# hyeeiin/ECG-Multimodal-Model

Hardware: AMD Instinct MI355X
Metric: samples/sec fwd+bwd, batch-256 multimodal (img+sig+clin), 1->8 MI355X (higher is better)
Workload: dtype bf16; 1 GPU; full multimodal (image 3x224x224 + 5000-pt signal + 16-dim clinical), fwd+bwd+Adam, encoders unfrozen; image_hw=224x224, per_gpu_batch=256, global_batch=256, parallelism=dp1

## Files before the change

### ecg-multimodal-model_amd/csrc/api.hip

```cpp
#include <stdarg.h>

#include "ops.h"

static thread_local char g_err[512] = "";

void ecg_set_error(const char* fmt, ...) {
  va_list ap;
  va_start(ap, fmt);
  vsnprintf(g_err, sizeof(g_err), fmt, ap);
  va_end(ap);
}

static inline ConvGeom geom_of(const ecgmm_conv_desc* c) {
  return make_geom(c->N, c->H, c->W, c->Cin, c->Cout, c->R, c->S, c->stride, c->pad_h, c->pad_w);
}
#define S_(x) ((hipStream_t)(x))

extern "C" {

int ecgmm_version(void) { return ECGMM_VERSION; }
const char* ecgmm_last_error(void) { return g_err; }

const char* ecgmm_switch_name(int i) { return i >= 0 && i < sw::COUNT ? sw::ALL[i]->env : nullptr; }
int ecgmm_switch_get(const char* env_name, int64_t* value) {
  Switch* s = sw::find(env_name);
  if (!s) ECG_FAIL(ECGMM_ERR_SHAPE, "switch_get: unknown switch %s", env_name ? env_name : "(null)");
  if (!value) ECG_FAIL(ECGMM_ERR_SHAPE, "switch_get: null value pointer");
  *value = s->get();
  return 0;
}
int ecgmm_switch_set(const char* env_name, int64_t value) {
  Switch* s = sw::find(env_name);
  if (!s) ECG_FAIL(ECGMM_ERR_SHAPE, "switch_set: unknown switch %s", env_name ? env_name : "(null)");
  if (s == &sw::SIDE_WGRAD)
    ECG_FAIL(ECGMM_ERR_SHAPE, "switch_set: ECGMM_SIDE_WGRAD is each plan's own state after start-up, call ecgmm_side_wgrad()");
  if (!s->runtime) ECG_FAIL(ECGMM_ERR_SHAPE, "switch_set: %s is read once at start-up", s->env);
  s->set((long)value);
  return 0;
}
int ecgmm_conv_halo_enable(int on) { sw::CONV_HALO.set(on); return 0; }
int ecgmm_conv_halo_cus(int cus) { sw::HALO_CUS.set(cus); return 0; }
int ecgmm_conv_halo_w4(int on) { sw::HALO_W4.set(on); return 0; }
int ecgmm_conv_halo_stagger(int on) { sw::HALO_STAGGER.set(on); return 0; }
int ecgmm_conv_halo_stream(int on) { sw::HALO_STREAM.set(on); return 0; }
int ecgmm_conv_halo_pingpong(int on) { sw::HALO_PP.set(on); return 0; }
int ecgmm_conv_wgrad_pingpong(int on) { sw::WGRAD_PP.set(on); return 0; }
int ecgmm_conv_wgrad_ring_enable(int on) { sw::WGRAD_RING.set(on); return 0; }
int ecgmm_bn_fold(int on) { sw::BN_FOLD.set(on); return 0; }
int ecgmm_bn_fold_slice(int on) { sw::BN_FOLD_SLICE.set(on); return 0; }
int ecgmm_bn_fuse_min_pixels(int64_t m) { sw::BN_FUSE_MIN_M.set((long)m); return 0; }
int ecgmm_stem_recompute(int on) { sw::STEM_RECOMPUTE.set(on); return 0; }
int ecgmm_infer_down_side(int on) { sw::INFER_DOWN_SIDE.set(on); return 0; }

int ecgmm_nchw_to_nhwc(int dtype, const float* src, void* dst, int N, int C, int64_t HW, void* stream) {
  return ecg_nchw_to_nhwc(dtype, src, dst, N, C, (long)HW, S_(stream));
}
int ecgmm_nhwc_to_nchw(int dtype, const void* src, float* dst, int N, int C, int64_t HW, void* stream) {
  return ecg_nhwc_to_nchw(dtype, src, dst, N, C, (long)HW, S_(stream));
}
int ecgmm_cast(int dtype, const float* src, void* dst, int64_t n, void* stream) {
  return ecg_cast(dtype, src, dst, (long)n, S_(stream));
}
int ecgmm_uncast(int dtype, const void* src, float* dst, int64_t n, void* stream) {
  return ecg_uncast(dtype, src, dst, (long)n, S_(stream));
}
int ecgmm_pack_conv_weight(int dtype, const float* w, void* fwd, void* dgrad, int Cout, int Cin, int RS,
                           void* stream) {
  return ecg_pack_weight(dtype, w, fwd, dgrad, Cout, Cin, RS, S_(stream));
}

int ecgmm_conv_stats_rows(int64_t out_pixels) { return ecg_conv_stats_rows((long)out_pixels); }
int ecgmm_conv_fwd(int dtype, const ecgmm_conv_desc* c, const void* x, const void* w_fwd, const float* bias, void* y,
                   float* stats, int act, void* stream) {
  return ecg_conv_igemm(dtype, 0, geom_of(c), x, w_fwd, y, bias, nullptr, stats, act, S_(stream));
}
int ecgmm_conv_bwd_data(int dtype, const ecgmm_conv_desc* c, const void* dy, const void* w_dgrad, const void* addend,
                        void* dx, void* stream) {
  return ecg_conv_igemm(dtype, 1, geom_of(c), dy, w_dgrad, dx, nullptr, addend, nullptr, 0, S_(stream));
}
size_t ecgmm_conv_bwd_weight_workspace(int dtype, const ecgmm_conv_desc* c) {
  return ecg_conv_wgrad_workspace(dtype, geom_of(c));
}
int ecgmm_conv_bwd_weight(int dtype, const ecgmm_conv_desc* c, const void* x, const void* dy, float* dw, int accumulate,
                          void* ws, size_t ws_bytes, void* stream) {
  return ecg_conv_wgrad(dtype, geom_of(c), x, dy, dw, accumulate, ws, ws_bytes, S_(stream));
}

size_t ecgmm_stem_packed_elems(int Cin, int R) { return ecg_stem_packed_elems(Cin, R); }
int ecgmm_stem_stats_rows(int N, int Cin, int H, int W, int R) { return ecg_stem_stats_rows(N, Cin, H, W, R); }
int ecgmm_stem_pack(int dtype, const float* w, void* packed, int Cin, int R, void* stream) {
  return ecg_stem_pack(dtype, w, packed, Cin, R, S_(stream));
}
int ecgmm_stem_fwd(int dtype, const float* x, const void* packed, const float* bias, void* y, float* stats, int N,
// ... 319 lines not shown
```

### ecg-multimodal-model_amd/csrc/conv_igemm.hip

```cpp
#include "ops.h"

namespace {

template <typename T> struct Mma;
template <> struct Mma<bf16_t> {
  static __device__ __forceinline__ void run(f32x4& acc, const u32x4& a, const u32x4& b) {
    acc = __builtin_amdgcn_mfma_f32_16x16x32_bf16(__builtin_bit_cast(bf16x8_t, a), __builtin_bit_cast(bf16x8_t, b),
                                                  acc, 0, 0, 0);
  }
};
template <> struct Mma<float> {
  static __device__ __forceinline__ void run(f32x4& acc, const u32x4& a, const u32x4& b) {
#pragma unroll
    for (int j = 0; j < 4; ++j)
      acc = __builtin_amdgcn_mfma_f32_16x16x4f32(__uint_as_float(a[j]), __uint_as_float(b[j]), acc, 0, 0, 0);
  }
};

__device__ __forceinline__ void dma16(__amdgpu_buffer_rsrc_t rs, unsigned char* lds_wave_base, unsigned voffset) {
#if defined(__HIP_DEVICE_COMPILE__)
  __builtin_amdgcn_raw_ptr_buffer_load_lds(rs, (__attribute__((address_space(3))) void*)lds_wave_base, 16, voffset, 0, 0,
                                           0);
#endif
}
// ... 514 lines not shown
static inline double conv_flops(const ConvGeom& g) {
  return 2.0 * (double)g.N * g.OH * g.OW * g.Cout * g.R * g.S * g.Cin;
}

int ecg_conv_igemm(int dtype, int mode, const ConvGeom& g, const void* src, const void* wpk, void* dst,
                   const float* bias, const void* addend, float* stats, int act, hipStream_t stream, ConvEpi* epi) {
  IgemmParams p;
  memset(&p, 0, sizeof(p));
  p.src = src; p.wpk = wpk; p.dst = dst; p.bias = bias; p.addend = addend; p.stats = stats; p.act = act;
  p.Nimg = g.N; p.R = g.R; p.S = g.S; p.stride = g.stride; p.pad_h = g.pad_h; p.pad_w = g.pad_w;
  if (mode == 0) {
    p.Hs = g.H; p.Ws = g.W; p.Cs = g.Cin; p.Hd = g.OH; p.Wd = g.OW; p.Cd = g.Cout;
  } else {
    p.Hs = g.OH; p.Ws = g.OW; p.Cs = g.Cout; p.Hd = g.H; p.Wd = g.W; p.Cd = g.Cin;
  }
  long M = (long)g.N * p.Hd * p.Wd;
  if (M <= 0 || M > 0x7fffffffL) ECG_FAIL(ECGMM_ERR_SHAPE, "conv: pixel count %ld out of range", M);
  {
    auto magic = [](unsigned d, unsigned& m, unsigned& sh) {
      if (d < 1) d = 1;
      int l = 0;
      while ((1u << l) < d) ++l;
      m = (unsigned)(((1ull << (31 + l)) + d - 1) / d);
      sh = 31 + l;
    };
    const bool par = mode == 1 && g.stride == 2;
    for (int c = 0; c < 4; ++c) {
      const int ph_ = par ? c >> 1 : 0, pw_ = par ? c & 1 : 0;
      const int Hc_ = par ? (p.Hd - ph_ + 1) >> 1 : p.Hd, Wc_ = par ? (p.Wd - pw_ + 1) >> 1 : p.Wd;
      magic((unsigned)(Hc_ * Wc_), p.mul_hw[c], p.sh_hw[c]);
      magic((unsigned)Wc_, p.mul_w[c], p.sh_w[c]);
    }
  }
  p.M = (int)M;
  const int vec = dtype == ECGMM_BF16 ? 8 : 4;
  if (p.Cs % vec != 0) ECG_FAIL(ECGMM_ERR_SHAPE, "conv: reduction channels %d not a multiple of %d", p.Cs, vec);
  if (dtype != ECGMM_BF16 && dtype != ECGMM_F32) ECG_FAIL(ECGMM_ERR_DTYPE, "conv: bad dtype %d", dtype);
  {
    const double esz = (double)dtype_size(dtype);
    double bytes = esz * ((double)g.N * p.Hs * p.Ws * p.Cs + (double)M * p.Cd * (addend ? 2.0 : 1.0) +
                          (double)g.R * g.S * g.Cin * g.Cout);
    if (epi && epi->red_y) bytes += esz * (double)M * p.Cd * (epi->red_mask ? 2.0 : 1.0);
    if (epi && epi->src2 && mode == 1 && g.stride == 2) bytes += esz * ((double)g.N * p.Hs * p.Ws * p.Cs + (double)g.Cin * g.Cout);
    ecg_prof_begin(dtype == ECGMM_F32 ? (mode == 0 ? ECG_PROF_IGEMM_F32_FWD : ECG_PROF_IGEMM_F32_DGRAD)
                                      : (mode == 0 ? ECG_PROF_IGEMM_FWD : ECG_PROF_IGEMM_DGRAD),
                   conv_flops(g), bytes, stream);
  }
  if (epi) epi->src2_done = 0;
  if (epi && epi->src2 && mode == 1 && g.stride == 2 && g.pad_h <= 1 && g.pad_w <= 1 && !addend) {
    p.src2 = epi->src2; p.wpk2 = epi->wpk2;
    epi->src2_done = 1;
  }
  int rc;
  if (ecg_conv_halo_ok(dtype, mode, g)) {
    rc = ecg_conv_halo(mode, g, src, wpk, dst, bias, addend, stats, act, epi, stream);
  } else {
    if (epi) {
      epi->stats_rows = ecg_conv_stats_rows(M);
      epi->red_done = 0;
      epi->red_rows_n = 0;
    }
    rc = dtype == ECGMM_BF16 ? launch_T<bf16_t>(p, mode, stream) : launch_T<float>(p, mode, stream);
  }
  ecg_prof_end(stream);
  return rc;
}
```

### ecg-multimodal-model_amd/csrc/ops.h

```cpp
#pragma once
#include "common.h"
#include "switches.h"

int ecg_conv_stats_rows(long M);
struct ConvEpi {
  const void* red_y;
  const void* red_mask;
  const float* red_coef;
  float* red_rows;
  int wg_rows;
  const void* src2;
  const void* wpk2;
  int src2_done;
  int stats_rows;
  int red_done;
  int red_rows_n;
};
int ecg_conv_igemm(int dtype, int mode, const ConvGeom& g, const void* src, const void* wpk, void* dst,
                   const float* bias, const void* addend, float* stats, int act, hipStream_t stream,
                   ConvEpi* epi = nullptr);
bool ecg_conv_halo_ok(int dtype, int mode, const ConvGeom& g);
int ecg_conv_halo_rows(int mode, const ConvGeom& g);
int ecg_conv_halo(int mode, const ConvGeom& g, const void* src, const void* wpk, void* dst, const float* bias,
                  const void* addend, float* stats, int act, ConvEpi* epi, hipStream_t stream);
size_t ecg_conv_wgrad_workspace(int dtype, const ConvGeom& g);
void ecg_conv_wgrad_narrow(bool narrow, int slots = 256);
int ecg_conv_wgrad(int dtype, const ConvGeom& g, const void* x, const void* dy, float* grad_oihw, int accumulate,
                   void* workspace, size_t workspace_bytes, hipStream_t stream);
size_t ecg_stem_packed_elems(int Cin, int R);
int ecg_stem_stats_rows(int N, int Cin, int H, int W, int R);
int ecg_stem_pack(int dtype, const float* w, void* out, int Cin, int R, hipStream_t stream);
int ecg_stem_fwd(int dtype, const float* x, const void* wpk, const float* bias, void* y, float* stats, int N, int Cin,
                 int H, int W, int R, hipStream_t stream);
size_t ecg_stem_wgrad_workspace(int N, int Cin, int H, int W, int R);
int ecg_stem_wgrad(int dtype, const float* x, const void* dy, float* grad, int accumulate, void* workspace,
                   size_t workspace_bytes, int N, int Cin, int H, int W, int R, hipStream_t stream);
int ecg_stem_stats_only_rows(int N, int Cin, int H, int W, int R);
int ecg_stem_wg_stats_rows(int N, int Cin, int H, int W, int R);
int ecg_stem_fwd_wgrows(int dtype, const float* x, const void* wpk, const float* bias, void* y, float* stats, int N, int Cin,
                        int H, int W, int R, hipStream_t stream);
int ecg_stem_stats_only(int dtype, const float* x, const void* wpk, const float* bias, float* stats, int N, int Cin, int H,
                        int W, int R, hipStream_t stream);
int ecg_stem_wgrad_reduce(const float* slab, float* grad, int rows, int NG, int accumulate, hipStream_t stream);
int ecg_stem_dgrad(int dtype, const void* dy, const float* w, float* dx, int N, int Cin, int H, int W, int R,
                   hipStream_t stream);
bool ecg_stem_fused_ok(int dtype, int Cin, int R);
int ecg_stem_pool_fwd(const float* x, const void* wpk, const float* coef, void* pooled, unsigned char* idx, int N, int Cin,
                      int H, int W, hipStream_t stream);
size_t ecg_stem_pool_bwd_workspace(int N, int Cin, int H, int W);
int ecg_stem_pool_bwd(const float* x, const void* wpk, const float* coef, const float* gamma, const void* dp, const void* pooled,
                      const unsigned char* idx, float* dgamma, float* dbeta, float* dw, void* ws, size_t ws_bytes, int N,
                      int Cin, int H, int W, hipStream_t stream);
int ecg_pool_bn_bwd_reduce(int dtype, const void* dp, const void* pooled, const float* coef, const float* gamma, float* dgamma,
                           float* dbeta, int N, int H, int W, int C, float* scratch, const float** bcoef_out,
                           hipStream_t stream);
int ecg_bn_rows(int dtype, long M, int C);
int ecg_bn_finalize(const float* partial, int rows, int C, double count, const float* gamma, const float* beta,
                    float* rm, float* rv, long long* nbt, float momentum, float eps, float* coef, hipStream_t stream);
int ecg_bn_eval_coef(int C, const float* gamma, const float* beta, const float* rm, const float* rv, float eps,
                     float* coef, hipStream_t stream);
int ecg_col_stats(int dtype, const void* x, long M, int C, float* partial, int* rows_out, hipStream_t stream);
struct EcgBnFold {
  const float* partial; int rows; double count;
  const float* gamma; const float* beta;
  float* rm; float* rv; long long* nbt;
  float momentum, eps;
};
bool ecg_bn_fold_ok(int C, int rows);
int ecg_bn_act_fold(int dtype, const void* y, float* coef, const EcgBnFold& f, const void* res, const float* rcoef,
                    const float* gate, int rows_per_sample, int relu, void* out, long M, int C, hipStream_t stream,
                    unsigned char* relu_bits = nullptr);
int ecg_bn_act(int dtype, const void* y, const float* coef, const void* res, const float* rcoef, const float* gate,
               int rows_per_sample, int relu, void* out, long M, int C, hipStream_t stream, unsigned char* relu_bits = nullptr);
size_t ecg_bn_bwd_scratch(int dtype, long M, int C);
int ecg_bn_bwd(int dtype, const void* dout, const void* maskref, const float* gate, const float* addc,
               int rows_per_sample, const void* y, const float* coef, const float* gamma, float* dgamma, float* dbeta,
               void* dy, void* dz_out, float* dbias, long M, int C, float* scratch, hipStream_t stream,
// ... 170 lines not shown
```

### ecg-multimodal-model_amd/hip/lib.py

```python
import ctypes as C
import os

F32, BF16 = 0, 1
ACT_NONE, ACT_RELU, ACT_SIGMOID = 0, 1, 2
RESNET18_NPARAMS, RESNET18_NBUFFERS = 62, 60
RESNET1D_NPARAMS, RESNET1D_NBUFFERS = 52, 27

_PKG_DIR = os.path.dirname(os.path.dirname(os.path.abspath(__file__)))
LIB_PATH = os.environ.get("ECGMM_LIB") or os.path.join(_PKG_DIR, "libecgmm_hip.so")

vp, i32, i64, u64, f32, f64, sz = C.c_void_p, C.c_int, C.c_int64, C.c_uint64, C.c_float, C.c_double, C.c_size_t


class ConvDesc(C.Structure):
    _fields_ = [(n, i32) for n in ("N", "H", "W", "Cin", "Cout", "R", "S", "stride", "pad_h", "pad_w")]


class ResNet18Desc(C.Structure):
    _fields_ = [("N", i32), ("H", i32), ("W", i32), ("out_dim", i32), ("dtype", i32), ("training", i32),
                ("bn_momentum", f32), ("bn_eps", f32)]


class ResNet1DDesc(C.Structure):
    _fields_ = [("N", i32), ("cin", i32), ("L", i32), ("num_classes", i32), ("dtype", i32), ("training", i32),
                ("bn_momentum", f32), ("bn_eps", f32), ("dropout_p", f32), ("seed", u64), ("offset", u64)]


class HeadDesc(C.Structure):
    _fields_ = [("B", i32), ("dim", i32 * 3), ("hidden", i32), ("num_classes", i32), ("training", i32),
                ("ln_eps", f32), ("dropout_p", f32), ("seed", u64), ("offset", u64)]


class LSTMDesc(C.Structure):
    _fields_ = [(n, i32) for n in ("B", "T", "In", "H", "layers", "bidirectional", "batch_first", "save_for_backward")]


class CRNNFrontDesc(C.Structure):
    _fields_ = [("B", i32), ("F", i32), ("T", i32), ("dtype", i32), ("training", i32), ("bn_momentum", f32), ("bn_eps", f32)]


P = C.POINTER
SIGNATURES = {
    "ecgmm_version": (i32, []),
    "ecgmm_last_error": (C.c_char_p, []),
    "ecgmm_switch_name": (C.c_char_p, [i32]),
    "ecgmm_switch_get": (i32, [C.c_char_p, P(i64)]),
    "ecgmm_switch_set": (i32, [C.c_char_p, i64]),
    "ecgmm_resnet18_fwd_workspace": (sz, [P(ResNet18Desc)]),
    "ecgmm_resnet18_bwd_workspace": (sz, [P(ResNet18Desc)]),
    "ecgmm_resnet18_forward": (i32, [P(ResNet18Desc), vp, P(vp), P(vp), vp, vp, sz, vp]),
    "ecgmm_resnet18_backward": (i32, [P(ResNet18Desc), vp, vp, P(vp), P(vp), vp, vp, sz, i32, i32, vp]),
    "ecgmm_resnet18_backward_dx": (i32, [P(ResNet18Desc), vp, vp, P(vp), P(vp), vp, vp, sz, i32, i32, vp, vp]),
    "ecgmm_resnet18_gradcam": (i32, [P(ResNet18Desc), vp, P(vp), vp, vp, sz, vp, vp]),
    "ecgmm_head_fwd_workspace": (sz, [P(HeadDesc)]),
    "ecgmm_head_bwd_workspace": (sz, [P(HeadDesc)]),
    "ecgmm_head_forward": (i32, [P(HeadDesc), P(vp), P(vp), P(vp), vp, vp, vp, sz, vp]),
    "ecgmm_head_backward": (i32, [P(HeadDesc), P(vp), P(vp), P(vp), P(vp), vp, P(vp), vp, vp, sz, vp]),
    "ecgmm_conv_halo_enable": (i32, [i32]),
    "ecgmm_conv_halo_cus": (i32, [i32]),
    "ecgmm_conv_halo_w4": (i32, [i32]),
    "ecgmm_conv_halo_stagger": (i32, [i32]),
    "ecgmm_conv_halo_stream": (i32, [i32]),
    "ecgmm_conv_halo_pingpong": (i32, [i32]),
    "ecgmm_conv_wgrad_pingpong": (i32, [i32]),
    "ecgmm_conv_wgrad_ring_enable": (i32, [i32]),
    "ecgmm_side_wgrad": (i32, [i32]),
    "ecgmm_side_defer_join": (i32, [i32]),
    "ecgmm_resnet1d_side_wgrad": (i32, [i32]),
    "ecgmm_side_wait": (i32, [vp]),
    "ecgmm_side_stream": (vp, []),
    "ecgmm_side_fork": (i32, [vp]),
    "ecgmm_resnet1d_fwd_workspace": (sz, [P(ResNet1DDesc)]),
    "ecgmm_resnet1d_bwd_workspace": (sz, [P(ResNet1DDesc)]),
    "ecgmm_resnet1d_forward": (i32, [P(ResNet1DDesc), vp, P(vp), P(vp), vp, vp, sz, vp]),
    "ecgmm_resnet1d_backward": (i32, [P(ResNet1DDesc), vp, vp, P(vp), P(vp), vp, vp, sz, i32, i32, vp]),
    "ecgmm_resnet1d_backward_dx": (i32, [P(ResNet1DDesc), vp, vp, P(vp), P(vp), vp, vp, sz, i32, i32, vp, vp]),
    "ecgmm_resnet1d_gradcam": (i32, [P(ResNet1DDesc), vp, P(vp), vp, vp, sz, vp, vp]),
    "ecgmm_nchw_to_nhwc": (i32, [i32, vp, vp, i32, i32, i64, vp]),
    "ecgmm_nhwc_to_nchw": (i32, [i32, vp, vp, i32, i32, i64, vp]),
    "ecgmm_cast": (i32, [i32, vp, vp, i64, vp]),
    "ecgmm_uncast": (i32, [i32, vp, vp, i64, vp]),
    "ecgmm_pack_conv_weight": (i32, [i32, vp, vp, vp, i32, i32, i32, vp]),
    "ecgmm_conv_stats_rows": (i32, [i64]),
    "ecgmm_conv_fwd": (i32, [i32, P(ConvDesc), vp, vp, vp, vp, vp, i32, vp]),
    "ecgmm_conv_fwd_wgrows": (i32, [i32, P(ConvDesc), vp, vp, vp, vp, vp, vp, i32, vp]),
    "ecgmm_conv_bwd_data": (i32, [i32, P(ConvDesc), vp, vp, vp, vp, vp]),
    "ecgmm_conv_bwd_weight_workspace": (sz, [i32, P(ConvDesc)]),
    "ecgmm_conv_bwd_weight": (i32, [i32, P(ConvDesc), vp, vp, vp, i32, vp, sz, vp]),
    "ecgmm_stem_packed_elems": (sz, [i32, i32]),
    "ecgmm_stem_stats_rows": (i32, [i32, i32, i32, i32, i32]),
    "ecgmm_stem_pack": (i32, [i32, vp, vp, i32, i32, vp]),
    "ecgmm_stem_fwd": (i32, [i32, vp, vp, vp, vp, vp, i32, i32, i32, i32, i32, vp]),
    "ecgmm_stem_wg_stats_rows": (i32, [i32, i32, i32, i32, i32]),
    "ecgmm_stem_fwd_wgrows": (i32, [i32, vp, vp, vp, vp, vp, i32, i32, i32, i32, i32, vp]),
    "ecgmm_stem_stats_only_rows": (i32, [i32, i32, i32, i32, i32]),
    "ecgmm_stem_stats_only": (i32, [i32, vp, vp, vp, vp, i32, i32, i32, i32, i32, vp]),
    "ecgmm_stem_pool_fwd": (i32, [vp, vp, vp, vp, vp, i32, i32, i32, i32, vp]),
    "ecgmm_stem_pool_bwd_workspace": (sz, [i32, i32, i32, i32]),
    "ecgmm_stem_pool_bwd": (i32, [vp, vp, vp, vp, vp, vp, vp, vp, vp, vp, vp, sz, i32, i32, i32, i32, vp]),
    "ecgmm_stem_bwd_weight_workspace": (sz, [i32, i32, i32, i32, i32]),
    "ecgmm_stem_bwd_weight": (i32, [i32, vp, vp, vp, i32, vp, sz, i32, i32, i32, i32, i32, vp]),
    "ecgmm_stem_bwd_data": (i32, [i32, vp, vp, vp, i32, i32, i32, i32, i32, vp]),
    "ecgmm_col_stats_rows": (i32, [i32, i64, i32]),
    "ecgmm_col_stats": (i32, [i32, vp, i64, i32, vp, vp]),
    "ecgmm_bn_finalize": (i32, [vp, i32, i32, f64, vp, vp, vp, vp, vp, f32, f32, vp, vp]),
    "ecgmm_bn_eval_coef": (i32, [i32, vp, vp, vp, vp, f32, vp, vp]),
    "ecgmm_bn_act": (i32, [i32, vp, vp, vp, vp, vp, i32, i32, vp, i64, i32, vp]),
    "ecgmm_bn_act_from_rows": (i32, [i32, vp, vp, i32, f64, vp, vp, vp, vp, vp, f32, f32, vp, vp, vp, vp, i32, i32, vp, i64, i32, vp]),
    "ecgmm_bn_bwd_scratch": (sz, [i32, i64, i32]),
    "ecgmm_bn_bwd": (i32, [i32, vp, vp, vp, vp, i32, vp, vp, vp, vp, vp, vp, vp, vp, i64, i32, vp, vp]),
    "ecgmm_bn_eval_bwd": (i32, [i32, vp, vp, vp, vp, i32, vp, vp, vp, vp, vp, vp, vp, i64, i32, vp, vp]),
# ... 37 lines not shown
    "ecgmm_signal_preprocess": (i32, [vp, vp, i32, i32, vp, vp, i32, P(f64), P(f64), P(f64), i32, vp, sz, vp]),
    "ecgmm_signal_filter_zscore": (i32, [vp, vp, i32, i32, P(f64), P(f64), P(f64), i32, i32, f64, vp]),
    "ecgmm_signal_gather_augment": (i32, [vp, i64, i32, vp, i32, vp, vp, i32, f32, f32, f32, f32, i32, i32, u64, u64, vp]),
    "ecgmm_glu_fwd": (i32, [vp, vp, i64, i32, vp]),
    "ecgmm_glu_bwd": (i32, [vp, vp, vp, i64, i32, vp]),
    "ecgmm_sparsemax_fwd": (i32, [vp, vp, i64, i32, vp]),
    "ecgmm_sparsemax_bwd": (i32, [vp, vp, vp, i64, i32, vp]),
    "ecgmm_ew": (i32, [i32, vp, vp, vp, i64, f32, vp]),
    "ecgmm_split_cols": (i32, [vp, vp, vp, i64, i32, i32, i32, vp]),
    "ecgmm_split_cols_bwd": (i32, [vp, vp, vp, vp, i64, i32, i32, i32, vp]),
    "ecgmm_bn_small_fwd": (i32, [vp, vp, vp, vp, vp, vp, vp, vp, i32, i32, i32, f32, f32, vp]),
    "ecgmm_bn_small_bwd": (i32, [vp, vp, vp, vp, vp, vp, vp, i32, i32, i32, vp]),
    "ecgmm_bn_small_eval_bwd": (i32, [vp, vp, vp, vp, vp, vp, vp, i32, i32, i32, vp]),
    "ecgmm_entropy_fwd": (i32, [vp, vp, i64, i32, f32, vp]),
    "ecgmm_entropy_bwd": (i32, [vp, vp, vp, i64, i32, f32, vp]),
    "ecgmm_image_resize_tables_bytes": (sz, [i32, i32, i32, i32]),
    "ecgmm_image_resize_tables": (i32, [i32, i32, i32, i32, vp, sz]),
    "ecgmm_image_transform": (i32, [vp, vp, i32, i32, i32, i32, i32, vp, sz, P(f32), P(f32), vp]),
    "ecgmm_resnet18_infer_prepared_bytes": (sz, [P(ResNet18Desc)]),
    "ecgmm_resnet18_infer_prepare": (i32, [P(ResNet18Desc), P(vp), P(vp), vp, sz, vp]),
    "ecgmm_resnet18_infer_workspace": (sz, [P(ResNet18Desc)]),
    "ecgmm_resnet18_infer": (i32, [P(ResNet18Desc), vp, vp, sz, vp, vp, sz, vp]),
    "ecgmm_resnet1d_infer_prepared_bytes": (sz, [P(ResNet1DDesc)]),
    "ecgmm_resnet1d_infer_prepare": (i32, [P(ResNet1DDesc), P(vp), P(vp), vp, sz, vp]),
    "ecgmm_resnet1d_infer_workspace": (sz, [P(ResNet1DDesc)]),
    "ecgmm_resnet1d_infer": (i32, [P(ResNet1DDesc), vp, vp, sz, vp, vp, sz, vp]),
    "ecgmm_infer_down_side": (i32, [i32]),
    "ecgmm_conv_fwd_fused": (i32, [i32, P(ConvDesc), vp, vp, vp, vp, vp, i32, vp]),
    "ecgmm_fold_conv_bn": (i32, [i32, i32, vp, vp, vp, vp, vp, vp, f32, vp, vp, vp, i32, i32, i32, vp]),
    "ecgmm_relu_maxpool": (i32, [i32, vp, vp, i32, i32, i32, i32, vp]),
    "ecgmm_gate_res_relu": (i32, [i32, vp, vp, vp, vp, i64, i32, i32, vp]),
    "ecgmm_prof_enable": (i32, [i32]),
    "ecgmm_prof_pause": (i32, [i32]),
    "ecgmm_prof_collect": (i32, [i32, P(f64), P(f64), P(f64), P(i64)]),
    "ecgmm_lstm_fwd_workspace": (sz, [P(LSTMDesc)]),
    "ecgmm_lstm_bwd_workspace": (sz, [P(LSTMDesc)]),
    "ecgmm_lstm_forward": (i32, [P(LSTMDesc), vp, P(vp), vp, vp, vp, vp, vp, vp, sz, vp]),
    "ecgmm_lstm_backward": (i32, [P(LSTMDesc), vp, P(vp), vp, vp, vp, vp, vp, vp, vp, P(vp), vp, vp, vp, sz, vp]),
    "ecgmm_conv5_in1_stats_rows": (i32, [i32, i32, i32]),
    "ecgmm_conv5_in1_fwd": (i32, [i32, vp, vp, vp, vp, vp, i32, i32, i32, vp]),
    "ecgmm_conv5_in1_bwd_weight_workspace": (sz, [i32, i32, i32]),
    "ecgmm_conv5_in1_bwd_weight": (i32, [i32, vp, vp, vp, vp, i32, vp, sz, i32, i32, i32, vp]),
    "ecgmm_conv5_bwd_weight_workspace": (sz, [i32, P(ConvDesc)]),
    "ecgmm_conv5_bwd_weight": (i32, [i32, P(ConvDesc), vp, vp, vp, i32, vp, sz, vp]),
    "ecgmm_bnrelu_maxpool2": (i32, [i32, vp, vp, vp, vp, i32, i32, i32, i32, i32, vp]),
    "ecgmm_pool2_bn_bwd_workspace": (sz, [i32, i32, i32, i32]),
    "ecgmm_pool2_bn_bwd": (i32, [i32, vp, vp, vp, vp, i32, vp, vp, vp, vp, i32, i32, i32, i32, i32, vp, sz, vp]),
    "ecgmm_crnn_front_fwd_workspace": (sz, [P(CRNNFrontDesc)]),
    "ecgmm_crnn_front_bwd_workspace": (sz, [P(CRNNFrontDesc)]),
    "ecgmm_crnn_front_forward": (i32, [P(CRNNFrontDesc), vp, P(vp), P(vp), vp, vp, sz, vp]),
    "ecgmm_crnn_front_backward": (i32, [P(CRNNFrontDesc), vp, vp, P(vp), P(vp), vp, vp, sz, vp]),
}

LATER_SYMBOLS = ("ecgmm_resnet18_backward_dx", "ecgmm_resnet18_gradcam", "ecgmm_resnet1d_backward_dx",
                 "ecgmm_resnet1d_gradcam", "ecgmm_stem_bwd_data", "ecgmm_bn_eval_bwd", "ecgmm_bn_small_eval_bwd",
                 "ecgmm_resnet18_infer_prepared_bytes", "ecgmm_resnet18_infer_prepare", "ecgmm_resnet18_infer_workspace",
                 "ecgmm_resnet18_infer", "ecgmm_resnet1d_infer_prepared_bytes", "ecgmm_resnet1d_infer_prepare",
                 "ecgmm_resnet1d_infer_workspace", "ecgmm_resnet1d_infer", "ecgmm_infer_down_side", "ecgmm_conv_fwd_fused",
                 "ecgmm_fold_conv_bn", "ecgmm_relu_maxpool", "ecgmm_gate_res_relu",
                 "ecgmm_signal_filter_zscore", "ecgmm_signal_gather_augment",
                 "ecgmm_lstm_fwd_workspace", "ecgmm_lstm_bwd_workspace", "ecgmm_lstm_forward", "ecgmm_lstm_backward",
                 "ecgmm_conv5_in1_stats_rows", "ecgmm_conv5_in1_fwd", "ecgmm_conv5_in1_bwd_weight_workspace",
                 "ecgmm_conv5_in1_bwd_weight", "ecgmm_conv5_bwd_weight_workspace", "ecgmm_conv5_bwd_weight",
                 "ecgmm_bnrelu_maxpool2", "ecgmm_pool2_bn_bwd_workspace", "ecgmm_pool2_bn_bwd",
                 "ecgmm_crnn_front_fwd_workspace", "ecgmm_crnn_front_bwd_workspace", "ecgmm_crnn_front_forward",
                 "ecgmm_crnn_front_backward",
                 "ecgmm_switch_name", "ecgmm_switch_get", "ecgmm_switch_set")

_lib = None


def _missing(name):
    def fail(*_a):
        raise RuntimeError(f"{LIB_PATH} does not export {name}: rebuild the HIP library (there is no fallback)")
    return fail


def lib():
    global _lib
    if _lib is None:
        if not os.path.exists(LIB_PATH):
            raise RuntimeError(
                f"libecgmm_hip.so not found at {LIB_PATH}: the HIP extension is the only compute path "
                "(no CPU fallback). Build it with `python __graft_entry__.py` or "
                "`make -C ecg-multimodal-model_amd/csrc`.")
        import torch
        h = C.CDLL(LIB_PATH)
        for name, (res, args) in SIGNATURES.items():
            if name in LATER_SYMBOLS and os.environ.get("ECGMM_LIB") and not hasattr(h, name):
                setattr(h, name, _missing(name))
                continue
            fn = getattr(h, name)
            fn.restype, fn.argtypes = res, args
        if h.ecgmm_version() != 100:
            raise RuntimeError(f"libecgmm_hip.so version {h.ecgmm_version()} != 100 (stale build?)")
        _lib = h
    return _lib


def check(rc, what=""):
    if rc != 0:
        msg = lib().ecgmm_last_error().decode(errors="replace")
        raise RuntimeError(f"ecgmm {what} failed (code {rc}): {msg}")
```

### include/ecgmm.h

```cpp
#ifndef ECGMM_H
#define ECGMM_H
#include <stddef.h>
#include <stdint.h>

#ifdef __cplusplus
extern "C" {
#endif

#define ECGMM_VERSION 100

enum { ECGMM_F32 = 0, ECGMM_BF16 = 1 };
enum { ECGMM_ACT_NONE = 0, ECGMM_ACT_RELU = 1, ECGMM_ACT_SIGMOID = 2 };
enum {
  ECGMM_OK = 0,
  ECGMM_ERR_SHAPE = 1,
  ECGMM_ERR_DTYPE = 2,
  ECGMM_ERR_WORKSPACE = 3,
  ECGMM_ERR_LAUNCH = 4
};

int ecgmm_version(void);
const char* ecgmm_last_error(void);

const char* ecgmm_switch_name(int i);
// ... 51 lines not shown
                            size_t ws_bwd_bytes, int stage_begin, int stage_end, void* stream);
int ecgmm_resnet1d_backward_dx(const ecgmm_resnet1d_desc* d, const float* signal, const float* dfeat,
                               const void* const* params, void* const* grads, void* ws_fwd, void* ws_bwd,
                               size_t ws_bwd_bytes, int stage_begin, int stage_end, float* dsignal, void* stream);
int ecgmm_resnet1d_gradcam(const ecgmm_resnet1d_desc* d, const float* dfeat, const void* const* params, void* ws_fwd,
                           void* ws_bwd, size_t ws_bwd_bytes, float* cam, void* stream);

size_t ecgmm_resnet18_infer_prepared_bytes(const ecgmm_resnet18_desc* d);
int ecgmm_resnet18_infer_prepare(const ecgmm_resnet18_desc* d, const void* const* params, const void* const* buffers,
                                 void* blob, size_t blob_bytes, void* stream);
size_t ecgmm_resnet18_infer_workspace(const ecgmm_resnet18_desc* d);
int ecgmm_resnet18_infer(const ecgmm_resnet18_desc* d, const float* image, const void* blob, size_t blob_bytes,
                         float* feat_out, void* ws, size_t ws_bytes, void* stream);
size_t ecgmm_resnet1d_infer_prepared_bytes(const ecgmm_resnet1d_desc* d);
int ecgmm_resnet1d_infer_prepare(const ecgmm_resnet1d_desc* d, const void* const* params, const void* const* buffers,
                                 void* blob, size_t blob_bytes, void* stream);
size_t ecgmm_resnet1d_infer_workspace(const ecgmm_resnet1d_desc* d);
int ecgmm_resnet1d_infer(const ecgmm_resnet1d_desc* d, const float* signal, const void* blob, size_t blob_bytes,
                         float* feat_out, void* ws, size_t ws_bytes, void* stream);
int ecgmm_infer_down_side(int on);

#define ECGMM_HEAD_NPARAMS 19
typedef struct {
  int B;
  int dim[3];
  int hidden;
  int num_classes;
  int training;
  float ln_eps;
  float dropout_p;
  uint64_t seed, offset;
} ecgmm_head_desc;
size_t ecgmm_head_fwd_workspace(const ecgmm_head_desc* d);
size_t ecgmm_head_bwd_workspace(const ecgmm_head_desc* d);
int ecgmm_head_forward(const ecgmm_head_desc* d, const float* const* raw, const void* const* params,
                       float* const* logits, float* var_loss, float* soft_w, void* ws, size_t ws_bytes, void* stream);
int ecgmm_head_backward(const ecgmm_head_desc* d, const float* const* raw, const void* const* params,
                        void* const* grads, const float* const* dlogits, const float* dvar, float* const* draw,
                        void* ws_fwd, void* ws_bwd, size_t ws_bwd_bytes, void* stream);

typedef struct {
  int N, H, W, Cin, Cout, R, S, stride, pad_h, pad_w;
} ecgmm_conv_desc;

int ecgmm_nchw_to_nhwc(int dtype, const float* src, void* dst, int N, int C, int64_t HW, void* stream);
int ecgmm_nhwc_to_nchw(int dtype, const void* src, float* dst, int N, int C, int64_t HW, void* stream);
int ecgmm_cast(int dtype, const float* src, void* dst, int64_t n, void* stream);
int ecgmm_uncast(int dtype, const void* src, float* dst, int64_t n, void* stream);
int ecgmm_pack_conv_weight(int dtype, const float* w_oihw, void* fwd, void* dgrad, int Cout, int Cin, int RS,
                           void* stream);

int ecgmm_conv_stats_rows(int64_t out_pixels);
int ecgmm_conv_halo_enable(int on);
int ecgmm_conv_halo_cus(int cus);
int ecgmm_conv_halo_w4(int on);
int ecgmm_conv_halo_stagger(int on);
int ecgmm_conv_halo_stream(int on);
int ecgmm_conv_halo_pingpong(int on);
int ecgmm_conv_wgrad_pingpong(int on);
int ecgmm_conv_wgrad_ring_enable(int on);
int ecgmm_conv_fwd(int dtype, const ecgmm_conv_desc* c, const void* x, const void* w_fwd, const float* bias, void* y,
                   float* stats, int act, void* stream);
int ecgmm_conv_fwd_wgrows(int dtype, const ecgmm_conv_desc* c, const void* x, const void* w_fwd, const float* bias, void* y,
                          float* stats, int* nrows, int act, void* stream);
int ecgmm_conv_bwd_data(int dtype, const ecgmm_conv_desc* c, const void* dy, const void* w_dgrad, const void* addend,
                        void* dx, void* stream);
size_t ecgmm_conv_bwd_weight_workspace(int dtype, const ecgmm_conv_desc* c);
int ecgmm_conv_bwd_weight(int dtype, const ecgmm_conv_desc* c, const void* x, const void* dy, float* dw_oihw,
                          int accumulate, void* ws, size_t ws_bytes, void* stream);

size_t ecgmm_stem_packed_elems(int Cin, int R);
int ecgmm_stem_stats_rows(int N, int Cin, int H, int W, int R);
int ecgmm_stem_pack(int dtype, const float* w_oihw, void* packed, int Cin, int R, void* stream);
int ecgmm_stem_fwd(int dtype, const float* x, const void* packed, const float* bias, void* y, float* stats, int N,
                   int Cin, int H, int W, int R, void* stream);
int ecgmm_stem_wg_stats_rows(int N, int Cin, int H, int W, int R);
int ecgmm_stem_fwd_wgrows(int dtype, const float* x, const void* packed, const float* bias, void* y, float* stats, int N,
                          int Cin, int H, int W, int R, void* stream);
size_t ecgmm_stem_bwd_weight_workspace(int N, int Cin, int H, int W, int R);
int ecgmm_stem_bwd_weight(int dtype, const float* x, const void* dy, float* dw_oihw, int accumulate, void* ws,
                          size_t ws_bytes, int N, int Cin, int H, int W, int R, void* stream);
int ecgmm_stem_bwd_data(int dtype, const void* dy, const float* w_oihw, float* dx, int N, int Cin, int H, int W, int R,
                        void* stream);

int ecgmm_stem_stats_only_rows(int N, int Cin, int H, int W, int R);
int ecgmm_stem_stats_only(int dtype, const float* x, const void* packed, const float* bias, float* stats, int N, int Cin,
                          int H, int W, int R, void* stream);
int ecgmm_stem_pool_fwd(const float* x, const void* packed, const float* coef, void* pooled, uint8_t* idx, int N, int Cin,
                        int H, int W, void* stream);
size_t ecgmm_stem_pool_bwd_workspace(int N, int Cin, int H, int W);
int ecgmm_stem_pool_bwd(const float* x, const void* packed, const float* coef, const float* gamma, const void* dp,
                        const void* pooled, const uint8_t* idx, float* dgamma, float* dbeta, float* dw_oihw, void* ws,
                        size_t ws_bytes, int N, int Cin, int H, int W, void* stream);

#define ECGMM_BN_TAIL_ROWS 64
int ecgmm_col_stats_rows(int dtype, int64_t M, int C);
int ecgmm_col_stats(int dtype, const void* x, int64_t M, int C, float* partial, void* stream);
int ecgmm_bn_finalize(const float* partial, int rows, int C, double count, const float* gamma, const float* beta,
                      float* running_mean, float* running_var, int64_t* num_batches_tracked, float momentum, float eps,
                      float* coef, void* stream);
int ecgmm_bn_eval_coef(int C, const float* gamma, const float* beta, const float* running_mean,
                       const float* running_var, float eps, float* coef, void* stream);
int ecgmm_bn_act(int dtype, const void* y, const float* coef, const void* res, const float* rcoef, const float* gate,
                 int rows_per_sample, int relu, void* out, int64_t M, int C, void* stream);
int ecgmm_bn_act_from_rows(int dtype, const void* y, const float* partial, int rows, double count, const float* gamma,
                           const float* beta, float* running_mean, float* running_var, int64_t* num_batches_tracked,
// ... 176 lines not shown
```

Baseline: 40140 samples/s.

## Add dedicated stride-2 dgrad kernel with halo tile and phase-class decomposition

Adds a specialised backward-data kernel for stride-2 3x3 (and 1x3 for 1D) convolutions. It splits output pixels into parity classes, so each class uses only its valid taps, and keeps a halo'd dy tile plus triple-buffered weight slices in LDS. The optional 1x1 downsample dgrad is fused in as an extra step. It is enabled by default at level 1, only for the Cs=128, Cd=64 shape, and only when there is no bias, addend, stats or activation. This aims to avoid the zero-tap waste of the generic implicit-GEMM path, at the cost of a large LDS footprint and new, less-tested code.

```diff
diff --git a/ecg-multimodal-model_amd/csrc/api.hip b/ecg-multimodal-model_amd/csrc/api.hip
--- a/ecg-multimodal-model_amd/csrc/api.hip
+++ b/ecg-multimodal-model_amd/csrc/api.hip
@@ -39,6 +39,7 @@
   return 0;
 }
 int ecgmm_conv_halo_enable(int on) { sw::CONV_HALO.set(on); return 0; }
+int ecgmm_conv_s2_halo(int level) { return ecg_conv_s2dgrad_level(level); }
 int ecgmm_conv_halo_cus(int cus) { sw::HALO_CUS.set(cus); return 0; }
 int ecgmm_conv_halo_w4(int on) { sw::HALO_W4.set(on); return 0; }
 int ecgmm_conv_halo_stagger(int on) { sw::HALO_STAGGER.set(on); return 0; }
diff --git a/ecg-multimodal-model_amd/csrc/conv_igemm.hip b/ecg-multimodal-model_amd/csrc/conv_igemm.hip
--- a/ecg-multimodal-model_amd/csrc/conv_igemm.hip
+++ b/ecg-multimodal-model_amd/csrc/conv_igemm.hip
@@ -590,7 +590,14 @@
     epi->src2_done = 1;
   }
   int rc;
-  if (ecg_conv_halo_ok(dtype, mode, g)) {
+  if (!bias && !addend && !stats && act == 0 && ecg_conv_s2dgrad_ok(dtype, mode, g)) {
+    if (epi) {
+      epi->stats_rows = ecg_conv_stats_rows(M);
+      epi->red_done = 0;
+      epi->red_rows_n = 0;
+    }
+    rc = ecg_conv_s2dgrad(g, src, wpk, p.src2, p.wpk2, dst, stream);
+  } else if (ecg_conv_halo_ok(dtype, mode, g)) {
     rc = ecg_conv_halo(mode, g, src, wpk, dst, bias, addend, stats, act, epi, stream);
   } else {
     if (epi) {
diff --git a/ecg-multimodal-model_amd/csrc/conv_s2dgrad.hip b/ecg-multimodal-model_amd/csrc/conv_s2dgrad.hip
--- /dev/null
+++ b/ecg-multimodal-model_amd/csrc/conv_s2dgrad.hip
@@ -0,0 +1,326 @@
+#include "ops.h"
+
+namespace {
+
+constexpr int S2T = 128;
+constexpr int S2_HCAP = 192;
+constexpr unsigned S2_OOB = 0x80000000u;
+
+struct S2Params {
+  const void* src;
+  const void* wpk;
+  const void* src2;
+  const void* wpk2;
+  void* dst;
+  int Ms;
+  int Hs, Ws, Hd, Wd, Cs, Cd;
+  int hrows;
+  int ntm;
+  int ntn;
+  unsigned mul_hw, sh_hw, mul_w, sh_w;
+};
+
+template <int NCS> struct S2Cfg {
+  static constexpr int PLANE = (S2_HCAP + 8) * 128;
+  static constexpr int S2B = NCS * PLANE;
+  static constexpr int S2PLANE = S2T * 128;
+  static constexpr int WB = S2B + NCS * S2PLANE;
+  static constexpr int WPLANE = 64 * 128;
+  static constexpr int WSLOT = NCS * WPLANE;
+  static constexpr int NWS = 3;
+  static constexpr int LDS = WB + NWS * WSLOT;
+};
+
+__device__ __forceinline__ void s2dma16(__amdgpu_buffer_rsrc_t rs, unsigned char* lds_wave_base, unsigned voffset,
+                                        unsigned soffset) {
+#if defined(__HIP_DEVICE_COMPILE__)
+  __builtin_amdgcn_raw_ptr_buffer_load_lds(rs, (__attribute__((address_space(3))) void*)lds_wave_base, 16, voffset,
+                                           soffset, 0, 0);
+#endif
+}
+template <int N> __device__ __forceinline__ void s2_wait_vmcnt() {
+#if defined(__HIP_DEVICE_COMPILE__)
+  asm volatile("s_waitcnt vmcnt(%0)" ::"n"(N) : "memory");
+#endif
+}
+__device__ __forceinline__ void s2_wait_lds() {
+#if defined(__HIP_DEVICE_COMPILE__)
+  __builtin_amdgcn_s_waitcnt(0xC07F);
+#endif
+}
+
+struct S2Step { int grp, cls, tap; };
+template <bool TWO_D> constexpr S2Step s2_step(int s) {
+  constexpr S2Step t2[10] = {{0, 3, 0}, {1, 3, 2}, {1, 2, 1}, {2, 3, 6}, {2, 1, 3}, {3, 3, 8}, {3, 2, 7}, {3, 1, 5}, {3, 0, 4}, {4, 0, 0}};
+  constexpr S2Step t1[4] = {{2, 1, 0}, {3, 1, 2}, {3, 0, 1}, {4, 0, 0}};
+  return TWO_D ? t2[s] : t1[s];
+}
+
+template <bool TWO_D, bool HAS2, int NCS>
+__global__ __launch_bounds__(512) void conv_s2dgrad_kernel(S2Params p) {
+  using C = S2Cfg<NCS>;
+  constexpr int NS = (TWO_D ? 9 : 3) + (HAS2 ? 1 : 0);
+  constexpr int NCL = TWO_D ? 4 : 2;
+  constexpr int NG = TWO_D ? 4 : 2;
+  constexpr int RS = TWO_D ? 9 : 3;
+  constexpr int TP = 2, TC = 2;
+  extern __shared__ __attribute__((aligned(16))) unsigned char smem[];
+
+  const int tid = threadIdx.x;
+  const int lane = tid & 63;
+  const int wv = __builtin_amdgcn_readfirstlane(tid >> 6);
+  const int wp = wv & 3, wc = wv >> 2;
+  const int fr = lane & 15, fq = lane >> 4;
+  const int nt = (int)blockIdx.x % p.ntn, kq = (int)blockIdx.x / p.ntn, Gk = (int)gridDim.x / p.ntn;
+  const int n0 = nt * 64;
+  const unsigned pixb = (unsigned)p.Cs * 2u;
+  const __amdgpu_buffer_rsrc_t rs_src = __builtin_amdgcn_make_buffer_rsrc((void*)p.src, 0, (int)((size_t)p.Ms * pixb), 0x00020000);
+  const __amdgpu_buffer_rsrc_t rs_src2 =
+      __builtin_amdgcn_make_buffer_rsrc((void*)(HAS2 ? p.src2 : p.src), 0, (int)((size_t)p.Ms * pixb), 0x00020000);
+  const __amdgpu_buffer_rsrc_t rs_w =
+      __builtin_amdgcn_make_buffer_rsrc((void*)p.wpk, 0, (int)((size_t)p.Cd * RS * pixb), 0x00020000);
+  const __amdgpu_buffer_rsrc_t rs_w2 =
+      __builtin_amdgcn_make_buffer_rsrc((void*)(HAS2 ? p.wpk2 : p.wpk), 0, (int)((size_t)p.Cd * pixb), 0x00020000);
+
+  const int lrow8 = lane >> 3;
+  const unsigned lchunkb = (unsigned)(((lane & 7) ^ lrow8) << 4);
+  const unsigned wrow = (unsigned)(n0 + wv * 8 + lrow8) * (unsigned)RS * pixb + lchunkb;
+  const unsigned wrow2 = (unsigned)(n0 + wv * 8 + lrow8) * pixb + lchunkb;
+  auto dma_w = [&](int s) {
+    const S2Step st = s2_step<TWO_D>(s);
+    unsigned char* slot = smem + C::WB + (s % C::NWS) * C::WSLOT + wv * 1024;
+#pragma unroll
+    for (int i = 0; i < NCS; ++i) {
+      if (st.grp == 4) s2dma16(rs_w2, slot + i * C::WPLANE, wrow2, (unsigned)i * 128u);
+      else s2dma16(rs_w, slot + i * C::WPLANE, wrow, (unsigned)st.tap * pixb + (unsigned)i * 128u);
+    }
+  };
+  auto dma_tile = [&](int m0) {
+#pragma unroll
+    for (int i = 0; i < 3 * NCS; ++i) {
+      const int plane = i / 3, pr = (i % 3) * 8 + wv;
+      const int row = pr * 8 + lrow8, pix = m0 + row;
+      const bool ok = row < p.hrows && pix < p.Ms;
+      s2dma16(rs_src, smem + plane * C::PLANE + pr * 1024, ok ? (unsigned)pix * pixb + lchunkb : S2_OOB, (unsigned)plane * 128u);
+    }
+    if (HAS2) {
+#pragma unroll
+      for (int i = 0; i < 2 * NCS; ++i) {
+        const int plane = i / 2, pr = (i % 2) * 8 + wv;
+        const int pix = m0 + pr * 8 + lrow8;
+        s2dma16(rs_src2, smem + C::S2B + plane * C::S2PLANE + pr * 1024, pix < p.Ms ? (unsigned)pix * pixb + lchunkb : S2_OOB,
+                (unsigned)plane * 128u);
+      }
+    }
+  };
+
+  unsigned aoff[TC];
+#pragma unroll
+  for (int a = 0; a < TC; ++a) {
+    const int row = wc * 32 + a * 16 + fr;
+    aoff[a] = (unsigned)C::WB + (unsigned)row * 128u + (unsigned)(((fq ^ row) & 7) << 4);
+  }
+  const unsigned zaddr = (unsigned)S2_HCAP * 128u + (unsigned)(fq << 4);
+  auto row_addr = [&](int R) -> unsigned { return (unsigned)R * 128u + (unsigned)(((fq ^ R) & 7) << 4); };
+
+  if (tid < 8 * NCS) *reinterpret_cast<u32x4*>(smem + (tid >> 3) * C::PLANE + S2_HCAP * 128 + (tid & 7) * 16) = (u32x4){0u, 0u, 0u, 0u};
+
+  bf16_t* __restrict__ dst = (bf16_t*)p.dst;
+  const int HWs = p.Hs * p.Ws;
+  int mt = kq;
+  if (mt < p.ntm) {
+    dma_tile(mt * S2T);
+    dma_w(0);
+    dma_w(1);
+  }
+  for (; mt < p.ntm; mt += Gk) {
+    const int m0 = mt * S2T;
+    unsigned baddr[TP][NG], s2addr[TP];
+    int opix[TP];
+    bool qok[TP], vr1[TP], vc1[TP];
+#pragma unroll
+    for (int b = 0; b < TP; ++b) {
+      const int pl = wp * 32 + b * 16 + fr;
+      const int q = m0 + pl;
+      qok[b] = q < p.Ms;
+      const int qq = qok[b] ? q : 0;
+      const int n = (int)(((unsigned long long)(unsigned)qq * p.mul_hw) >> p.sh_hw), rem = qq - n * HWs;
+      const int ai = (int)(((unsigned long long)(unsigned)rem * p.mul_w) >> p.sh_w), bi = rem - ai * p.Ws;
+      const bool r1 = TWO_D && ai + 1 < p.Hs, c1 = bi + 1 < p.Ws;
+#pragma unroll
+      for (int g = 0; g < NG; ++g) {
+        const int grp = TWO_D ? g : g + 2;
+        const int dr = grp < 2 ? 1 : 0, dc = (grp & 1) ? 0 : 1;
+        const bool ok = qok[b] && (dr == 0 || r1) && (dc == 0 || c1);
+        baddr[b][g] = ok ? row_addr(pl + dr * p.Ws + dc) : zaddr;
+      }
+      s2addr[b] = (unsigned)C::S2B + row_addr(pl);
+      opix[b] = (n * p.Hd + 2 * ai) * p.Wd + 2 * bi;
+      vr1[b] = 2 * ai + 1 < p.Hd;
+      vc1[b] = 2 * bi + 1 < p.Wd;
+    }
+    f32x4 acc[NCL][TC][TP];
+#pragma unroll
+    for (int c = 0; c < NCL; ++c)
+#pragma unroll
+      for (int a = 0; a < TC; ++a)
+#pragma unroll
+        for (int b = 0; b < TP; ++b) acc[c][a][b] = (f32x4){0.f, 0.f, 0.f, 0.f};
+
+    u32x4 fa[NCS][2][TC], fb[NCS][2][TP];
+#pragma unroll
+    for (int s = 0; s < NS; ++s) {
+      const S2Step st = s2_step<TWO_D>(s);
+      if (s == 0 || s + 1 >= NS) s2_wait_vmcnt<0>();
+      else s2_wait_vmcnt<NCS>();
+      s2_wait_lds();
+      __builtin_amdgcn_s_barrier();
+      if (s + 2 < NS) dma_w(s + 2);
+      if (s == 0 || st.grp != s2_step<TWO_D>(s > 0 ? s - 1 : 0).grp) {
+#pragma unroll
+        for (int cs = 0; cs < NCS; ++cs)
+#pragma unroll
+          for (int ks = 0; ks < 2; ++ks)
+#pragma unroll
+            for (int b = 0; b < TP; ++b) {
+              const unsigned ad = st.grp == 4 ? (s2addr[b] ^ (unsigned)(ks * 64)) + (unsigned)(cs * C::S2PLANE)
+                                              : (baddr[b][TWO_D ? st.grp : st.grp - 2] ^ (unsigned)(ks * 64)) + (unsigned)(cs * C::PLANE);
+              fb[cs][ks][b] = *reinterpret_cast<const u32x4*>(smem + ad);
+            }
+      }
+#pragma unroll
+      for (int cs = 0; cs < NCS; ++cs)
+#pragma unroll
+        for (int ks = 0; ks < 2; ++ks)
+#pragma unroll
+          for (int a = 0; a < TC; ++a)
+            fa[cs][ks][a] = *reinterpret_cast<const u32x4*>(smem + (aoff[a] ^ (unsigned)(ks * 64)) +
+                                                             (unsigned)((s % C::NWS) * C::WSLOT + cs * C::WPLANE));
+#pragma unroll
+      for (int cs = 0; cs < NCS; ++cs)
+#pragma unroll
+        for (int ks = 0; ks < 2; ++ks)
+#pragma unroll
+          for (int a = 0; a < TC; ++a)
+#pragma unroll
+            for (int b = 0; b < TP; ++b)
+              acc[st.cls][a][b] = __builtin_amdgcn_mfma_f32_16x16x32_bf16(__builtin_bit_cast(bf16x8_t, fa[cs][ks][a]),
+                                                                          __builtin_bit_cast(bf16x8_t, fb[cs][ks][b]),
+                                                                          acc[st.cls][a][b], 0, 0, 0);
+    }
+    s2_wait_lds();
+    __builtin_amdgcn_s_barrier();
+    if (mt + Gk < p.ntm) {
+      dma_tile((mt + Gk) * S2T);
+      dma_w(0);
+      dma_w(1);
+    }
+#if defined(__HIP_DEVICE_COMPILE__)
+#pragma unroll
+    for (int c = 0; c < NCL; ++c) {
+      const int ph = TWO_D ? c >> 1 : 0, pw = c & 1;
+#pragma unroll
+      for (int b = 0; b < TP; ++b) {
+        const f32x4 v0 = acc[c][0][b], v1 = acc[c][1][b];
+        const unsigned x0 = (unsigned)f2bf(v0[0]) | ((unsigned)f2bf(v0[1]) << 16);
+        const unsigned y0 = (unsigned)f2bf(v0[2]) | ((unsigned)f2bf(v0[3]) << 16);
+        const unsigned x1 = (unsigned)f2bf(v1[0]) | ((unsigned)f2bf(v1[1]) << 16);
+        const unsigned y1 = (unsigned)f2bf(v1[2]) | ((unsigned)f2bf(v1[3]) << 16);
+        auto lo = __builtin_amdgcn_permlane16_swap(x0, x1, false, false);
+        auto hi = __builtin_amdgcn_permlane16_swap(y0, y1, false, false);
+        const int ch = (fq & 1) ? 16 + (fq - 1) * 4 : fq * 4;
+        const bool ok = qok[b] && (ph == 0 || vr1[b]) && (pw == 0 || vc1[b]);
+        if (ok)
+          *reinterpret_cast<u32x4*>(dst + (size_t)(opix[b] + ph * p.Wd + pw) * p.Cd + n0 + wc * 32 + ch) =
+              (u32x4){lo[0], hi[0], lo[1], hi[1]};
+      }
+    }
+#endif
+  }
+}
+
+void s2_magic_div(unsigned d, unsigned& m, unsigned& sh) {
+  if (d < 1) d = 1;
+  int l = 0;
+  while ((1u << l) < d) ++l;
+  m = (unsigned)(((1ull << (31 + l)) + d - 1) / d);
+  sh = 31 + l;
+}
+
+int s2_cus() {
+  static int ncu[16] = {0};
+  int dev = 0;
+  (void)hipGetDevice(&dev);
+  if (dev < 0 || dev >= 16) return 256;
+  if (ncu[dev] == 0) {
+    hipDeviceProp_t prop;
+    ncu[dev] = hipGetDeviceProperties(&prop, dev) == hipSuccess && prop.multiProcessorCount > 0 ? prop.multiProcessorCount : 256;
+  }
+  return ncu[dev];
+}
+
+template <bool TWO_D, bool HAS2, int NCS>
+int launch_s2(const S2Params& p, hipStream_t stream) {
+  using C = S2Cfg<NCS>;
+  static bool attr_set[16] = {false};
+  int dev = 0;
+  (void)hipGetDevice(&dev);
+  if (dev >= 0 && dev < 16 && !attr_set[dev]) {
+    if (hipFuncSetAttribute((const void*)conv_s2dgrad_kernel<TWO_D, HAS2, NCS>, hipFuncAttributeMaxDynamicSharedMemorySize, C::LDS) !=
+        hipSuccess)
+      ECG_FAIL(ECGMM_ERR_LAUNCH, "conv_s2dgrad: cannot reserve %d bytes of LDS", C::LDS);
+    attr_set[dev] = true;
+  }
+  int Gk = s2_cus() / p.ntn;
+  if (Gk > p.ntm) Gk = p.ntm;
+  if (Gk < 1) Gk = 1;
+  hipLaunchKernelGGL((conv_s2dgrad_kernel<TWO_D, HAS2, NCS>), dim3(Gk * p.ntn), dim3(512), C::LDS, stream, p);
+  ECG_CHECK_LAUNCH("conv_s2dgrad_kernel");
+  return 0;
+}
+
+}
+
+static int g_s2_level = 1;
+int ecg_conv_s2dgrad_level(int level) {
+  const int old = g_s2_level;
+  if (level >= 0) g_s2_level = level > 2 ? 2 : level;
+  return old;
+}
+bool ecg_conv_s2dgrad_ok(int dtype, int mode, const ConvGeom& g) {
+  const int level = g_s2_level;
+  if (!level || dtype != ECGMM_BF16 || mode != 1 || g.stride != 2 || g.S != 3 || g.pad_w != 1) return false;
+  const bool two_d = g.R == 3 && g.pad_h == 1, one_d = g.R == 1 && g.pad_h == 0 && g.H == 1;
+  if (!two_d && !one_d) return false;
+  const int Cs = g.Cout, Cd = g.Cin;
+  if ((Cs != 64 && Cs != 128) || Cd % 64 != 0) return false;
+  if (g.W > 2 * g.OW || g.W < 2 * g.OW - 1) return false;
+  if (two_d && (g.H > 2 * g.OH || g.H < 2 * g.OH - 1)) return false;
+  if (S2T + (two_d ? g.OW : 0) + 1 > S2_HCAP) return false;
+  const double Ms = (double)g.N * g.OH * g.OW;
+  if (Ms < 1 || Ms * Cs * 2.0 > 2.0e9 || (double)g.N * g.H * g.W > 2.0e9) return false;
+  if (level == 2) return true;
+  return Cs == 128 && Cd == 64;
+}
+
+int ecg_conv_s2dgrad(const ConvGeom& g, const void* src, const void* wpk, const void* src2, const void* wpk2, void* dst,
+                     hipStream_t stream) {
+  S2Params p;
+  memset(&p, 0, sizeof(p));
+  p.src = src; p.wpk = wpk; p.src2 = src2; p.wpk2 = wpk2; p.dst = dst;
+  p.Hs = g.OH; p.Ws = g.OW; p.Hd = g.H; p.Wd = g.W; p.Cs = g.Cout; p.Cd = g.Cin;
+  p.Ms = g.N * g.OH * g.OW;
+  const bool two_d = g.R == 3;
+  p.hrows = S2T + (two_d ? g.OW : 0) + 1;
+  p.ntm = ceil_div(p.Ms, S2T);
+  p.ntn = p.Cd / 64;
+  s2_magic_div((unsigned)(p.Hs * p.Ws), p.mul_hw, p.sh_hw);
+  s2_magic_div((unsigned)p.Ws, p.mul_w, p.sh_w);
+  const bool has2 = src2 != nullptr;
+  if (p.Cs == 128) {
+    if (two_d) return has2 ? launch_s2<true, true, 2>(p, stream) : launch_s2<true, false, 2>(p, stream);
+    return has2 ? launch_s2<false, true, 2>(p, stream) : launch_s2<false, false, 2>(p, stream);
+  }
+  if (two_d) return has2 ? launch_s2<true, true, 1>(p, stream) : launch_s2<true, false, 1>(p, stream);
+  return has2 ? launch_s2<false, true, 1>(p, stream) : launch_s2<false, false, 1>(p, stream);
+}
diff --git a/ecg-multimodal-model_amd/csrc/ops.h b/ecg-multimodal-model_amd/csrc/ops.h
--- a/ecg-multimodal-model_amd/csrc/ops.h
+++ b/ecg-multimodal-model_amd/csrc/ops.h
@@ -23,6 +23,10 @@
 int ecg_conv_halo_rows(int mode, const ConvGeom& g);
 int ecg_conv_halo(int mode, const ConvGeom& g, const void* src, const void* wpk, void* dst, const float* bias,
                   const void* addend, float* stats, int act, ConvEpi* epi, hipStream_t stream);
+int ecg_conv_s2dgrad_level(int level);
+bool ecg_conv_s2dgrad_ok(int dtype, int mode, const ConvGeom& g);
+int ecg_conv_s2dgrad(const ConvGeom& g, const void* src, const void* wpk, const void* src2, const void* wpk2, void* dst,
+                     hipStream_t stream);
 size_t ecg_conv_wgrad_workspace(int dtype, const ConvGeom& g);
 void ecg_conv_wgrad_narrow(bool narrow, int slots = 256);
 int ecg_conv_wgrad(int dtype, const ConvGeom& g, const void* x, const void* dy, float* grad_oihw, int accumulate,
diff --git a/ecg-multimodal-model_amd/hip/lib.py b/ecg-multimodal-model_amd/hip/lib.py
--- a/ecg-multimodal-model_amd/hip/lib.py
+++ b/ecg-multimodal-model_amd/hip/lib.py
@@ -57,6 +57,7 @@
     "ecgmm_head_forward": (i32, [P(HeadDesc), P(vp), P(vp), P(vp), vp, vp, vp, sz, vp]),
     "ecgmm_head_backward": (i32, [P(HeadDesc), P(vp), P(vp), P(vp), P(vp), vp, P(vp), vp, vp, sz, vp]),
     "ecgmm_conv_halo_enable": (i32, [i32]),
+    "ecgmm_conv_s2_halo": (i32, [i32]),
     "ecgmm_conv_halo_cus": (i32, [i32]),
     "ecgmm_conv_halo_w4": (i32, [i32]),
     "ecgmm_conv_halo_stagger": (i32, [i32]),
@@ -200,7 +201,7 @@
     "ecgmm_crnn_front_backward": (i32, [P(CRNNFrontDesc), vp, vp, P(vp), P(vp), vp, vp, sz, vp]),
 }
 
-LATER_SYMBOLS = ("ecgmm_resnet18_backward_dx", "ecgmm_resnet18_gradcam", "ecgmm_resnet1d_backward_dx",
+LATER_SYMBOLS = ("ecgmm_conv_s2_halo", "ecgmm_resnet18_backward_dx", "ecgmm_resnet18_gradcam", "ecgmm_resnet1d_backward_dx",
                  "ecgmm_resnet1d_gradcam", "ecgmm_stem_bwd_data", "ecgmm_bn_eval_bwd", "ecgmm_bn_small_eval_bwd",
                  "ecgmm_resnet18_infer_prepared_bytes", "ecgmm_resnet18_infer_prepare", "ecgmm_resnet18_infer_workspace",
                  "ecgmm_resnet18_infer", "ecgmm_resnet1d_infer_prepared_bytes", "ecgmm_resnet1d_infer_prepare",
diff --git a/include/ecgmm.h b/include/ecgmm.h
--- a/include/ecgmm.h
+++ b/include/ecgmm.h
@@ -127,6 +127,7 @@
 
 int ecgmm_conv_stats_rows(int64_t out_pixels);
 int ecgmm_conv_halo_enable(int on);
+int ecgmm_conv_s2_halo(int level);
 int ecgmm_conv_halo_cus(int cus);
 int ecgmm_conv_halo_w4(int on);
 int ecgmm_conv_halo_stagger(int on);
```

After: 40310 samples/s (median of 6 runs). No clear change (+0.4%).
